# AlainSchoebi/semantic-bundle-adjustment-colmap

Hardware: AMD Instinct MI355X
Metric: residuals+Jacobians/sec and BA-iteration wall-time, 1k cams / 1M pts / 10M obs (higher is better)
Workload: dtype f64

## Files before the change

### semantic-bundle-adjustment-colmap_amd/csrc/semantic.hip

```cpp
#include <hip/hip_runtime.h>

#include <map>

#include <algorithm>
#include <cmath>
#include <cstring>
#include <type_traits>

#include "ba_math.h"
#include "kernels.h"
#include "semantic.h"
#include "step_bodies.h"

namespace miba {

namespace {

constexpr double kMinStep = 1.4901161193847656e-08;

struct SemArgs {
  const SemSample* samples;
  const SemPair* pairs;
  const double* qt;
  const double* cam;
// ... 147 lines not shown
  const double aa = a * a, bb = b * b, cc = c * c, dd = d * d;
  const double ab = a * b, ac = a * c, ad = a * d, bc = b * c, bd = b * d, cd = c * d;
  Q[0] = aa + bb - cc - dd; Q[1] = 2.0 * (bc - ad);  Q[2] = 2.0 * (ac + bd);
  Q[3] = 2.0 * (bc + ad);  Q[4] = aa - bb + cc - dd; Q[5] = 2.0 * (cd - ab);
  Q[6] = 2.0 * (bd - ac);  Q[7] = 2.0 * (ab + cd);  Q[8] = aa - bb - cc + dd;
}

[[maybe_unused]] __device__ inline double rcp_refined(double x) {
  double r = __builtin_amdgcn_rcp(x);
  r = fma(r, fma(-x, r, 1.0), r);
  r = fma(r, fma(-x, r, 1.0), r);
  return r;
}

template <int M>
__device__ inline double distortion_gain(const double* K, double r2) {
  constexpr int np = Model<M>::kNumParams;
  double s = 0.0;
  if constexpr (M == kSimpleRadial || M == kRadial) {
#pragma unroll
    for (int k = 3; k < np; ++k) s += fabs(K[k]);
  } else if constexpr (M == kOpenCV) {
#pragma unroll
    for (int k = 4; k < np; ++k) s += fabs(K[k]);
  }
  const double g = 1.0 + r2;
  return 1.0 + s * g * g * g;
}

template <int M>
__device__ inline void world_to_image_fma(const double* K, double u, double v, double* x, double* y) {
#pragma clang fp contract(fast)
  if constexpr (M == kSimplePinhole) {
    *x = K[0] * u + K[1];
    *y = K[0] * v + K[2];
  } else if constexpr (M == kPinhole) {
    *x = K[0] * u + K[2];
    *y = K[1] * v + K[3];
  } else if constexpr (M == kSimpleRadial || M == kRadial) {
    const double r2 = u * u + v * v;
    double rad = K[3] * r2;
    if constexpr (M == kRadial) rad = rad + K[4] * r2 * r2;
// ... 5 lines not shown
    const double rad = k1 * r2 + k2 * r2 * r2;
    const double du = u * rad + 2.0 * p1 * uv + p2 * (r2 + 2.0 * u2);
    const double dv = v * rad + 2.0 * p2 * uv + p1 * (r2 + 2.0 * v2);
    *x = K[0] * (u + du) + K[2];
    *y = K[1] * (v + dv) + K[3];
  }
}

__device__ inline void matvec3_t_fma(const double* A, double v0, double v1, double v2, const double* t,
                                     double pp[3]) {
#pragma clang fp contract(fast)
#pragma unroll
  for (int c = 0; c < 3; ++c) pp[c] = A[3 * c] * v0 + A[3 * c + 1] * v1 + A[3 * c + 2] * v2 + t[c];
}

template <int M>
__device__ inline double margin_model_term(const double* K2, const double p[3], double mag) {
  const double iz = 1.0 / p[2];
  const double u = p[0] * iz, v = p[1] * iz;
  return 2e-11 * (fabs(K2[0]) + fabs(K2[1])) * distortion_gain<M>(K2, u * u + v * v) * (1.0 + fabs(u) + fabs(v)) *
         (1.0 + mag * fabs(iz));
}

template <int M, bool FAST = false>
__device__ inline bool resolve(const SemArgs& a, const double p[3], double mag, float label1, const double* K2,
                               const float2* dl2, const PixelCache& pc, double& f, double exk = 0.0) {
  double iz;
  if constexpr (FAST) {
    const double x0 = p[2];
    double r = __builtin_amdgcn_rcp(x0);
    iz = fma(r, fma(-x0, r, 1.0), r);
  } else {
    iz = rcp_refined(p[2]);
  }
  const double u = p[0] * iz, v = p[1] * iz;
// ... 20 lines not shown
    f = 0.0;
    return true;
  }
  float2 s;
  if (pc.valid && px == pc.px && py == pc.py) {
    s = make_float2(pc.depth, pc.label);
  } else {
    s = dl2[(size_t)py * a.W + px];
  }
  const double dd = fabs((double)s.x - p[2]) - a.threshold;
  if (!(fabs(dd) > 1e-9 * (1.0 + fabs((double)s.x) + mag))) return false;
  f = (dd > 0.0) ? 0.0 : ((label1 == s.y) ? 0.0 : 1.0);
  return true;
}

struct PairConst {
  double q1[4], t1[3], q2[4], t2[3];
  double uqi[4];
  double ti[3];
  double u2[4];
  double R2[9];
  double C[9];
  double K2[8];
  uint32_t var1, var2, mask1, mask2;
  uint32_t slot, H2, W2, TW2;
  uint64_t roff, toff;
  double pert[28];
  double ood[14];
  double A[16][9];
  double pj[8][3];
  double rho1, rho2, dt1[3], dt2[3];
};

__device__ __forceinline__ SemArgs with_pair(const SemArgs& ak, const PairConst* __restrict__ P) {
  SemArgs a = ak;
  a.H = (int)P->H2;
  a.W = (int)P->W2;
  a.TW = (int)P->TW2;
  return a;
}

__device__ inline void stencil_bounds(const double* q, const double* t, double rel_step, double* rho, double dt[3]) {
  const double nq2 = q[0] * q[0] + q[1] * q[1] + q[2] * q[2] + q[3] * q[3];
  const double nq = sqrt(nq2);
  double r = 0.0;
  for (int k = 0; k < 4; ++k) {
    const double delta = fmax(kMinStep, fabs(q[k]) * rel_step);
    const double d = fmax(fabs((q[k] + delta) - q[k]), fabs(q[k] - (q[k] - delta)));
    const double perp = d * sqrt(fmax(0.0, 1.0 - q[k] * q[k] / nq2));
    const double den = nq - d;
    r = fmax(r, den > 0.0 ? 2.0 * perp / den : INFINITY);
  }
  *rho = r * 1.001;
  for (int k = 0; k < 3; ++k) {
    const double delta = fmax(kMinStep, fabs(t[k]) * rel_step);
    dt[k] = fmax(fabs((t[k] + delta) - t[k]), fabs(t[k] - (t[k] - delta))) * 1.001;
  }
}

__device__ inline void stencil_prep(const double* q1, const double* t1, const double* q2, const double* t2,
                                    double rel_step, int e, PairConst* __restrict__ P) {
  const int m = e >> 1;
  const bool minus = e & 1;
  const int grp = m < 4 ? 0 : (m < 7 ? 1 : (m < 11 ? 2 : 3));
  const int k = m - (grp == 0 ? 0 : (grp == 1 ? 4 : (grp == 2 ? 7 : 11)));
  const double orig = grp == 0 ? q1[k] : (grp == 1 ? t1[k] : (grp == 2 ? q2[k] : t2[k]));
  const double delta = fmax(kMinStep, fabs(orig) * rel_step);
  const double pert = minus ? orig - delta : orig + delta;
  P->pert[e] = pert;
  if (minus) {
    double one_over_delta = 1.0 / delta;
    one_over_delta /= 2;
// ... 28 lines not shown
      for (int kk = 1; kk < 4; ++kk) v = kk == k ? PJ[3 * kk + c] : v;
      P->pj[(grp == 0 ? 0 : 4) + k][c] = v;
    }
  }
}

constexpr int kPairVals = 78 + 12;
constexpr int kPairStride = 96;
constexpr int kSemRow = 13;

__device__ __forceinline__ void pair_prep_body(int k, int lane, const SemPair* __restrict__ pairs, int npairs,
                                      const double* __restrict__ qt, const double* __restrict__ cam,
                                      const uint32_t* __restrict__ img_cam, const uint32_t* __restrict__ img_flags,
                                      const uint32_t* __restrict__ raster_slot, const SlotInfo* __restrict__ slots,
                                      double rel_step, PairConst* __restrict__ out, double* __restrict__ pair_blk,
                                      int blk_stride, uint32_t* __restrict__ pair_cnt) {
  if (k >= npairs) return;
  for (int e = lane; e < blk_stride; e += 32) pair_blk[(size_t)k * blk_stride + e] = 0.0;
  if (pair_cnt && lane == 31) pair_cnt[k] = 0u;
  if (lane > 30) return;
  const SemPair pr = pairs[k];
  const double* a1 = qt + 8 * (size_t)pr.i;
  const double* a2 = qt + 8 * (size_t)pr.j;
  if (lane < 28) {
    stencil_prep(a1, a1 + 4, a2, a2 + 4, rel_step, lane, out + k);
    return;
  }
  PairConst& P = out[k];
  const double zero[3] = {0.0, 0.0, 0.0};
  if (lane == 28) {
    const double q1[4] = {a1[0], a1[1], a1[2], a1[3]}, t1[3] = {a1[4], a1[5], a1[6]};
    for (int m = 0; m < 4; ++m) P.q1[m] = q1[m];
    for (int m = 0; m < 3; ++m) P.t1[m] = t1[m];
    Pose1Stage s;
    pose1_stage(q1, zero, s);
    {
      const double sc = 1.0 / sqrt(q1[0] * q1[0] + q1[1] * q1[1] + q1[2] * q1[2] + q1[3] * q1[3]);
      const double qi[4] = {sc * q1[0], -(sc * q1[1]), -(sc * q1[2]), -(sc * q1[3])};
      const double scale = 1.0 / sqrt(qi[0] * qi[0] + qi[1] * qi[1] + qi[2] * qi[2] + qi[3] * qi[3]);
// ... 34 lines not shown
    double u2[4], R2[9];
    unit_quat(q2, u2);
    unit_quat_matrix(u2, R2);
    for (int r = 0; r < 3; ++r)
      for (int c = 0; c < 3; ++c)
        P.C[3 * r + c] = R2[3 * r] * s.R[c] + R2[3 * r + 1] * s.R[3 + c] + R2[3 * r + 2] * s.R[6 + c];
  }
}

__global__ void semantic_pair_prep_kernel(const SemPair* __restrict__ pairs, int npairs, const double* __restrict__ qt,
                                          const double* __restrict__ cam, const uint32_t* __restrict__ img_cam,
                                          const uint32_t* __restrict__ img_flags,
                                          const uint32_t* __restrict__ raster_slot,
                                          const SlotInfo* __restrict__ slots, double rel_step,
                                          PairConst* __restrict__ out, double* __restrict__ pair_blk, int blk_stride,
                                          uint32_t* __restrict__ pair_cnt, uint32_t* __restrict__ zero_n = nullptr,
                                          int nzero = 0) {
  if (zero_n && blockIdx.x == 0 && (int)threadIdx.x < nzero) zero_n[threadIdx.x] = 0u;
  pair_prep_body(blockIdx.x * 2 + (threadIdx.x >> 5), threadIdx.x & 31, pairs, npairs, qt, cam, img_cam, img_flags,
                 raster_slot, slots, rel_step, out, pair_blk, blk_stride, pair_cnt);
}

struct PrepArgs {
  const SemPair* pairs;
  int npairs;
  const double* qt;
  const double* cam;
  const uint32_t* img_cam;
  const uint32_t* img_flags;
  const uint32_t* raster_slot;
  const SlotInfo* slots;
  double rel_step;
  PairConst* out;
  double* pair_blk;
  uint32_t* pair_cnt;
  uint32_t* dcount;
};

template <int U>
__global__ __launch_bounds__(256, 8) void step_prologue_kernel(PrepArgs a, int nprep, DevProblem p,
                                                            double* __restrict__ rec, double* __restrict__ zero,
                                                            int nzero, int npack, TouchRanges t, unsigned* sink,
                                                            int nwarm) {
  const int b = blockIdx.x;
  if (b < nprep) {
    if (b == 0 && (int)threadIdx.x < kNumModels) a.dcount[threadIdx.x] = 0u;
    pair_prep_body(b * 8 + (threadIdx.x >> 5), threadIdx.x & 31, a.pairs, a.npairs, a.qt, a.cam, a.img_cam,
                   a.img_flags, a.raster_slot, a.slots, a.rel_step, a.out, a.pair_blk, kPairStride, a.pair_cnt);
  } else if (b < nprep + npack) {
    pack_image_record(p, rec, zero, nzero, (b - nprep) * 256 + (int)threadIdx.x);
  } else {
    touch_ranges<U>(t, sink, b - nprep - npack, nwarm);
  }
}


template <int M>
__device__ __forceinline__ double stencil_reference(const SemArgs& a, const PairConst* __restrict__ P, int grp, int k,
                                                 double pert, const double pc1[3], float label1, const double* K2,
                                                 const float2* dl2) {
  double qq1[4], tt1[3], qq2[4], tt2[3];
#pragma unroll
  for (int c = 0; c < 4; ++c) {
// ... 301 lines not shown
  }
  return ok;
}

struct Centre {
  double pw[3], p2[3], w[3];
  double r, mag, exk;
  PixelCache pc;
  int st;
};

template <int M, bool FAST>
__device__ __forceinline__ void centre_eval(const SemArgs& a, const PairConst* __restrict__ P, const SemSample& smp,
                                            const double* K2, const float2* dl2, Centre& c) {
  double rot[3];
  unit_quat_rotate(P->uqi, smp.pc1, rot);
  c.pw[0] = rot[0] + P->ti[0];
  c.pw[1] = rot[1] + P->ti[1];
  c.pw[2] = rot[2] + P->ti[2];
  double rot2[3];
  unit_quat_rotate(P->u2, c.pw, rot2);
  c.p2[0] = rot2[0] + P->t2[0];
  c.p2[1] = rot2[1] + P->t2[1];
  c.p2[2] = rot2[2] + P->t2[2];
  c.pc.valid = false;
  c.pc.px = c.pc.py = 0;
  c.pc.depth = c.pc.label = 0.f;
  c.st = 0;
  c.r = project_centre<M>(a, c.p2, smp.label1, K2, dl2, c.pc, &c.st);
  c.mag = fabs(smp.pc1[0]) + fabs(smp.pc1[1]) + fabs(smp.pc1[2]) + fabs(P->t1[0]) + fabs(P->t1[1]) +
          fabs(P->t1[2]) + fabs(c.pw[0]) + fabs(c.pw[1]) + fabs(c.pw[2]) + fabs(P->t2[0]) + fabs(P->t2[1]) +
          fabs(P->t2[2]);
  c.w[0] = smp.pc1[0] - P->t1[0];
  c.w[1] = smp.pc1[1] - P->t1[1];
  c.w[2] = smp.pc1[2] - P->t1[2];
  c.exk = FAST ? margin_model_term<M>(K2, c.p2, c.mag) : 0.0;
}

template <int M, bool FAST, int NB>
__device__ __forceinline__ bool stencil_full(const SemArgs& a, const PairConst* __restrict__ P, const Centre& c,
                                             const SemSample& smp, const double* K2, const float2* dl2,
                                             double Jt[12], const float2* box = nullptr,
                                             const FlatBox* fb = nullptr) {
  if constexpr (NB > 0) {
    const int cidx = c.pc.valid ? c.pc.py * a.W + c.pc.px : 0;
    if (!stencil_batched<M, FAST, NB>(a, P, c.w, c.pw, c.p2, c.mag, smp.label1, K2, dl2, cidx, c.exk, Jt, box, fb)) {
      stencil_rolled<M, FAST>(a, P, c.w, c.pw, c.p2, c.mag, smp.pc1, smp.label1, K2, dl2, c.pc, c.exk, Jt);
      return true;
    }
    return false;
  } else {
// ... 1 lines not shown
    return true;
  }
}


template <int M>
__device__ __forceinline__ double second_derivative_bound(const double* K, double rho) {
  if constexpr (M == kSimpleRadial) {
    return 6.0 * fabs(K[3]) * rho;
  } else if constexpr (M == kRadial) {
    return 6.0 * fabs(K[3]) * rho + 20.0 * fabs(K[4]) * rho * rho * rho;
  } else if constexpr (M == kOpenCV) {
    return 6.0 * fabs(K[4]) * rho + 20.0 * fabs(K[5]) * rho * rho * rho + 6.0 * (fabs(K[6]) + fabs(K[7]));
  } else {
    return 0.0;
  }
}

template <int M>
__device__ __forceinline__ bool flat_box(const PairConst* __restrict__ P, const Centre& c, const double* K2,
                                         FlatBox& fb) {
  const double z = c.p2[2];
  if (!(z > 0.0)) return false;
  const double iz = 1.0 / z;
  const double u = c.p2[0] * iz, v = c.p2[1] * iz;
  constexpr int np = Model<M>::kNumParams;
  double x, y, A[4], Jp[2 * np];
  world_to_image_jac<M>(K2, u, v, &x, &y, A, Jp);
  if (!(fabs(x) < 1e8 && fabs(y) < 1e8 && fabs(u) < 1e6 && fabs(v) < 1e6)) return false;
  const double dq1 = P->var1 ? P->rho1 * sqrt(c.w[0] * c.w[0] + c.w[1] * c.w[1] + c.w[2] * c.w[2]) * (1.0 + 1e-12) : 0.0;
// ... 38 lines not shown
  }
  const double gain = distortion_gain<M>(K2, u * u + v * v);
  const double kscale = (fabs(K2[0]) + fabs(K2[1])) * gain * (1.0 + fabs(u) + fabs(v)) * (1.0 + c.mag * fabs(iz));
  const double ex = 1e-6 + 1e-11 * (kscale + fabs(x) + fabs(y));
  const double bx = bxm * (1.0 + 1e-12) + ex;
  const double by = bym * (1.0 + 1e-12) + ex;
  fb.x0 = (int)round(x - bx);
  fb.y0 = (int)round(y - by);
  fb.ncol = (int)round(x + bx) - fb.x0 + 1;
  fb.nrow = (int)round(y + by) - fb.y0 + 1;
  fb.d = az_max;
  return fb.ncol <= 3 && fb.nrow <= 3;
}

template <int M>
__device__ __forceinline__ void image_jac_bound(const double* K, double u, double v, double Ah[4]) {
  const double r2 = u * u + v * v, r1 = fabs(u) + fabs(v);
  if constexpr (M == kSimplePinhole) {
    Ah[0] = Ah[3] = fabs(K[0]);
    Ah[1] = Ah[2] = 0.0;
  } else if constexpr (M == kPinhole) {
    Ah[0] = fabs(K[0]);
    Ah[3] = fabs(K[1]);
    Ah[1] = Ah[2] = 0.0;
  } else if constexpr (M == kSimpleRadial) {
    const double k = fabs(K[3]);
    Ah[0] = Ah[3] = fabs(K[0]) * (1.0 + 3.0 * k * r2);
    Ah[1] = Ah[2] = fabs(K[0]) * (k * r2);
  } else if constexpr (M == kRadial) {
    const double k1 = fabs(K[3]), k2 = fabs(K[4]);
    Ah[0] = Ah[3] = fabs(K[0]) * (1.0 + 3.0 * k1 * r2 + 5.0 * k2 * r2 * r2);
    Ah[1] = Ah[2] = fabs(K[0]) * (k1 * r2 + 2.0 * k2 * r2 * r2);
  } else {
    const double k1 = fabs(K[4]), k2 = fabs(K[5]), p1 = fabs(K[6]), p2 = fabs(K[7]);
    const double rad = 3.0 * k1 * r2 + 5.0 * k2 * r2 * r2, off = k1 * r2 + 2.0 * k2 * r2 * r2 + 2.0 * (p1 + p2) * r1;
    Ah[0] = fabs(K[0]) * (1.0 + rad + (2.0 * p1 + 6.0 * p2) * r1);
    Ah[1] = fabs(K[0]) * off;
    Ah[2] = fabs(K[1]) * off;
    Ah[3] = fabs(K[1]) * (1.0 + rad + (6.0 * p1 + 2.0 * p2) * r1);
  }
}

template <int M, bool EXACT_A = false, bool GROUPS = false>
__device__ __forceinline__ bool flat_box_coarse(const PairConst* __restrict__ P, const Centre& c, const double* K2,
                                                double u, double v, double x, double y, FlatBox& fb) {
  const double z = c.p2[2];
  if (!(z > 0.0)) return false;
  double Ae[4];
  if constexpr (EXACT_A) {
    constexpr int np = Model<M>::kNumParams;
    double Jp[2 * np];
    world_to_image_jac<M>(K2, u, v, &x, &y, Ae, Jp);
  }
  if (!(fabs(x) < 1e8 && fabs(y) < 1e8 && fabs(u) < 1e6 && fabs(v) < 1e6)) return false;
  double dq = 0.0, tx = 0.0, ty = 0.0, tz = 0.0;
  if (P->var1) {
    dq = P->rho1 * sqrt(c.w[0] * c.w[0] + c.w[1] * c.w[1] + c.w[2] * c.w[2]) * (1.0 + 1e-12);
    tx = fmax(P->dt1[0] * fabs(P->C[0]), fmax(P->dt1[1] * fabs(P->C[1]), P->dt1[2] * fabs(P->C[2])));
    ty = fmax(P->dt1[0] * fabs(P->C[3]), fmax(P->dt1[1] * fabs(P->C[4]), P->dt1[2] * fabs(P->C[5])));
    tz = fmax(P->dt1[0] * fabs(P->C[6]), fmax(P->dt1[1] * fabs(P->C[7]), P->dt1[2] * fabs(P->C[8])));
  }
  if (P->var2) {
    dq = fmax(dq, P->rho2 * sqrt(c.pw[0] * c.pw[0] + c.pw[1] * c.pw[1] + c.pw[2] * c.pw[2]) * (1.0 + 1e-12));
    tx = fmax(tx, P->dt2[0]);
    ty = fmax(ty, P->dt2[1]);
    tz = fmax(tz, P->dt2[2]);
  }
  const double az = fmax(dq, tz);
  if (!(z - az > 0.5 * z)) return false;
  const double iden = 1.0 / (z - az) * (1.0 + 1e-12);
  const double cu_r = (dq + fabs(u) * dq) * iden, cv_r = (dq + fabs(v) * dq) * iden;
  const double cu_t = (tx + fabs(u) * tz) * iden, cv_t = (ty + fabs(v) * tz) * iden;
  const double cu = fmax(cu_r, cu_t), cv = fmax(cv_r, cv_t);
  const double gm = fmax(cu, cv);
  if (!(gm < 0.1)) return false;
  const double ru = fabs(u) + gm, rv = fabs(v) + gm;
  const double H = second_derivative_bound<M>(K2, sqrt(ru * ru + rv * rv) * (1.0 + 1e-12));
  const double fx = fabs(K2[0]);
  const double fy = (M == kPinhole || M == kOpenCV) ? fabs(K2[1]) : fabs(K2[0]);
  double Ah[4];
  if constexpr (EXACT_A) {
#pragma unroll
    for (int k = 0; k < 4; ++k) Ah[k] = fabs(Ae[k]);
  } else {
    image_jac_bound<M>(K2, u, v, Ah);
  }
  double bxm, bym;
  if constexpr (GROUPS) {
    const double sr = cu_r + cv_r, st = cu_t + cv_t;
    bxm = fmax((Ah[0] + fx * H * sr) * cu_r + (Ah[1] + fx * H * sr) * cv_r,
               (Ah[0] + fx * H * st) * cu_t + (Ah[1] + fx * H * st) * cv_t);
    bym = fmax((Ah[2] + fy * H * sr) * cu_r + (Ah[3] + fy * H * sr) * cv_r,
               (Ah[2] + fy * H * st) * cu_t + (Ah[3] + fy * H * st) * cv_t);
  } else {
    const double sk = cu + cv;
    bxm = (Ah[0] + fx * H * sk) * cu + (Ah[1] + fx * H * sk) * cv;
    bym = (Ah[2] + fy * H * sk) * cu + (Ah[3] + fy * H * sk) * cv;
  }
  const double gain = distortion_gain<M>(K2, u * u + v * v);
  const double kscale = (fabs(K2[0]) + fabs(K2[1])) * gain * (1.0 + fabs(u) + fabs(v)) * (1.0 + c.mag * fabs(1.0 / z));
  const double ex = 1e-6 + 1e-11 * (kscale + fabs(x) + fabs(y));
  const double bx = bxm * (1.0 + 1e-12) + ex;
  const double by = bym * (1.0 + 1e-12) + ex;
  fb.x0 = (int)round(x - bx);
  fb.y0 = (int)round(y - by);
  fb.ncol = (int)round(x + bx) - fb.x0 + 1;
  fb.nrow = (int)round(y + by) - fb.y0 + 1;
  fb.d = az;
  return fb.ncol <= 3 && fb.nrow <= 3;
}

__device__ __forceinline__ int flat_index(const SemArgs& a, const FlatBox& fb, bool cand, int q) {
  const int px = fb.x0 + q % 3, py = fb.y0 + q / 3;
  const bool in = cand && q % 3 < fb.ncol && q / 3 < fb.nrow && px >= 0 && px < a.W && py >= 0 && py < a.H;
  return in ? py * a.W + px : 0;
// ... 270 lines not shown
  if (!(dmin <= dmax)) return 0;
  const double margin = fb.d + 1e-9 * (1.0 + fmax(fabs(dmin), fabs(dmax)) + mag);
  const double far = fmax(fabs(dmax - z), fabs(dmin - z));
  if (a.threshold - far > margin) return 1;
  const double nearest = (z >= dmin && z <= dmax) ? 0.0 : fmin(fabs(dmin - z), fabs(dmax - z));
  if (nearest - a.threshold > margin) return 2;
  return 0;
}

template <int M, bool WS, bool LP, int COARSE>
__device__ __forceinline__ double flat_sample(const SemArgs& a, const PairConst* __restrict__ P, const double* K2,
                                              const float2* dl2, const float* spal, const SemSample& smp, Centre& c,
                                              bool& deferred, bool& decided) {
  deferred = false;
  double rot[3];
  unit_quat_rotate(P->uqi, smp.pc1, rot);
  c.pw[0] = rot[0] + P->ti[0];
  c.pw[1] = rot[1] + P->ti[1];
  c.pw[2] = rot[2] + P->ti[2];
  double rot2[3];
  unit_quat_rotate(P->u2, c.pw, rot2);
  c.p2[0] = rot2[0] + P->t2[0];
  c.p2[1] = rot2[1] + P->t2[1];
  c.p2[2] = rot2[2] + P->t2[2];
  c.mag = fabs(smp.pc1[0]) + fabs(smp.pc1[1]) + fabs(smp.pc1[2]) + fabs(P->t1[0]) + fabs(P->t1[1]) +
          fabs(P->t1[2]) + fabs(c.pw[0]) + fabs(c.pw[1]) + fabs(c.pw[2]) + fabs(P->t2[0]) + fabs(P->t2[1]) +
          fabs(P->t2[2]);
  c.w[0] = smp.pc1[0] - P->t1[0];
  c.w[1] = smp.pc1[1] - P->t1[1];
  c.w[2] = smp.pc1[2] - P->t1[2];
  const double u2 = c.p2[0] / c.p2[2];
  const double v2 = c.p2[1] / c.p2[2];
  double x2, y2;
  world_to_image<M>(K2, u2, v2, &x2, &y2);
  const int cpx = cast_to_int_x86(round(x2));
  const int cpy = cast_to_int_x86(round(y2));
  const bool cin = !(cpx < 0 || cpx >= a.W || cpy < 0 || cpy >= a.H);
  FlatBox fb;
  const bool cand = COARSE == 3   ? flat_box_coarse<M, false, true>(P, c, K2, u2, v2, x2, y2, fb)
                    : COARSE == 2 ? flat_box_coarse<M, true>(P, c, K2, u2, v2, x2, y2, fb)
                    : COARSE == 1 ? flat_box_coarse<M>(P, c, K2, u2, v2, x2, y2, fb)
                                  : flat_box<M>(P, c, K2, fb);
  decided = false;
  bool resolved = false;
  if constexpr (LP) {
    if (cand && fb.x0 >= 0 && fb.y0 >= 0 && fb.x0 + fb.ncol <= a.W && fb.y0 + fb.nrow <= a.H && cpx >= fb.x0 &&
        cpx < fb.x0 + fb.ncol && cpy >= fb.y0 && cpy < fb.y0 + fb.nrow) {
      const float2 dr = a.dtile[P->toff + (size_t)(fb.y0 >> 3) * a.TW + (fb.x0 >> 3)];
      const uint8_t* lp = a.lab8 + P->roff + (size_t)fb.y0 * a.W + fb.x0;
// ... 35 lines not shown
    float2 s[9];
#pragma unroll
    for (int q = 0; q < 9; ++q) s[q] = dl2[flat_index(a, fb, cand, q)];
    if (!cin) {
      c.st = MI_BA_OUT_OF_BOUNDS;
      c.r = 0.0;
    } else if (fabs((double)sc.x - c.p2[2]) > a.threshold) {
      c.st = MI_BA_INVALID_DEPTH;
      c.r = 0.0;
    } else {
      c.st = MI_BA_VALID;
      c.r = (smp.label1 == sc.y) ? 0.0 : 1.0;
    }
    deferred = !(cand && flat_check(a, fb, s, c.p2[2], c.mag, smp.label1, c.r));
  }
  double rho[3];
  loss_eval(a.loss_type, a.loss_scale, c.r * c.r, rho);
  return 0.5 * (a.weight * rho[0]);
}

__device__ __forceinline__ void tile_cost_sum(double cost, double* sred, int tid, int lane, double* __restrict__ out) {
  double v = cost;
  for (int off = 32; off > 0; off >>= 1) v += __shfl_xor(v, off, 64);
  if (lane == 0) sred[tid >> 6] = v;
  __syncthreads();
  if (tid == 0) {
    double s = 0.0;
#pragma unroll
    for (int w = 0; w < kBlock / 64; ++w) s += sred[w];
    *out = s;
  }
}

// ... 124 lines not shown
        cb = 12;
      }
      double acc = 0.0;
      for (int q = 0; q < rows; ++q) acc += sJ[q * kSemRow + ca] * sJ[q * kSemRow + cb];
      cpart[((size_t)pair_chunk0[ch.x] + ch.y / 64) * kPairVals + e] = acc;
    }
  }
  __syncthreads();
  }
}

template <int M>
__device__ __forceinline__ void centre_geometry(const PairConst* __restrict__ P, const SemSample& smp,
                                                const double* K2, Centre& c) {
  double rot[3];
  unit_quat_rotate(P->uqi, smp.pc1, rot);
  c.pw[0] = rot[0] + P->ti[0];
  c.pw[1] = rot[1] + P->ti[1];
  c.pw[2] = rot[2] + P->ti[2];
  double rot2[3];
  unit_quat_rotate(P->u2, c.pw, rot2);
  c.p2[0] = rot2[0] + P->t2[0];
  c.p2[1] = rot2[1] + P->t2[1];
  c.p2[2] = rot2[2] + P->t2[2];
  c.pc.valid = false;
  c.pc.px = c.pc.py = 0;
  c.pc.depth = c.pc.label = 0.f;
  c.st = 0;
  c.r = 0.0;
  c.mag = fabs(smp.pc1[0]) + fabs(smp.pc1[1]) + fabs(smp.pc1[2]) + fabs(P->t1[0]) + fabs(P->t1[1]) +
          fabs(P->t1[2]) + fabs(c.pw[0]) + fabs(c.pw[1]) + fabs(c.pw[2]) + fabs(P->t2[0]) + fabs(P->t2[1]) +
          fabs(P->t2[2]);
  c.w[0] = smp.pc1[0] - P->t1[0];
  c.w[1] = smp.pc1[1] - P->t1[1];
  c.w[2] = smp.pc1[2] - P->t1[2];
  c.exk = margin_model_term<M>(K2, c.p2, c.mag);
}

template <int M, int GRP>
__device__ __forceinline__ bool stencil_group(const SemArgs& a, const PairConst* __restrict__ P, const Centre& c,
                                              const SemSample& smp, const double* K2, const float2* dl2,
                                              double col[3]) {
  constexpr int n = (GRP == 0 || GRP == 2) ? 4 : 3;
  constexpr int m0 = GRP == 0 ? 0 : (GRP == 1 ? 4 : (GRP == 2 ? 7 : 11));
  const uint32_t mask = GRP == 1 ? P->mask1 : (GRP == 3 ? P->mask2 : 0u);
  col[0] = col[1] = col[2] = 0.0;
  const PixelCache none = {0, 0, 0.f, 0.f, false};
  double fp[4], fm[4];
  const bool ok = stencil_step<M, true, GRP, 4>(a, P, m0, 0, n, c.w, c.pw, c.p2, c.mag, smp.label1, K2, dl2, 0, c.exk,
                                                fp, fm);
  if (ok) {
// ... 1079 lines not shown

void semantic_destroy(mi_ba_context* ctx) {
  if (!ctx->sem) return;
  delete ctx->sem;
  ctx->sem = nullptr;
}

mi_ba_status semantic_pair_prep(mi_ba_context* ctx, hipStream_t stream) {
  SemanticState* S = ctx->sem;
  if (!S || S->ns == 0 || S->npairs == 0) return MI_BA_OK;
  SemArgs a = make_args(ctx, ctx->dev.qt, ctx->dev.cam);
  PairConst* pcs = reinterpret_cast<PairConst*>(S->pconst.ptr);
  hipLaunchKernelGGL(semantic_pair_prep_kernel, dim3((S->npairs + 1) / 2), dim3(64), 0, stream, S->pairs.ptr,
                     S->npairs, a.qt, a.cam, a.img_cam, a.img_flags, a.raster_slot, a.slots, a.rel_step, pcs,
                     S->pair_blk.ptr,
                     kPairStride, ctx->sem_variant == 6 ? S->pair_cnt.ptr : nullptr,
                     ctx->sem_variant == 6 ? S->dcount.ptr : nullptr, kNumModels);
  return hipGetLastError() == hipSuccess ? MI_BA_OK : MI_BA_ERR_HIP;
}

mi_ba_status semantic_step_prologue(mi_ba_context* ctx, hipStream_t stream, double* zero, int nzero, unsigned* sink,
                                    int warm_mask, int warm_wgs, int warm_unroll) {
  SemanticState* S = ctx->sem;
  if (!S || S->ns == 0 || S->npairs == 0 || ctx->sem_variant != 6) return MI_BA_ERR_STATE;
  const DevProblem& d = ctx->dev;
  SemArgs a = make_args(ctx, d.qt, d.cam);
  PrepArgs pa{S->pairs.ptr, S->npairs, a.qt, a.cam, a.img_cam, a.img_flags, a.raster_slot, a.slots, a.rel_step,
              reinterpret_cast<PairConst*>(S->pconst.ptr), S->pair_blk.ptr, S->pair_cnt.ptr, S->dcount.ptr};
  const int nprep = (S->npairs + 7) / 8;
  const int npack = (int)((std::max<int64_t>(d.num_images, nzero) + 255) / 256);
  const int nwarm = touch_workgroups(warm_wgs);
  const TouchRanges t = touch_input_ranges(d, warm_mask);
  const dim3 grid((unsigned)(nprep + npack + nwarm));
  if (warm_unroll >= 8)
    hipLaunchKernelGGL(step_prologue_kernel<8>, grid, dim3(256), 0, stream, pa, nprep, d, ctx->img_rec.ptr, zero, nzero,
                       npack, t, sink, nwarm);
  else
    hipLaunchKernelGGL(step_prologue_kernel<4>, grid, dim3(256), 0, stream, pa, nprep, d, ctx->img_rec.ptr, zero, nzero,
                       npack, t, sink, nwarm);
  return hipGetLastError() == hipSuccess ? MI_BA_OK : MI_BA_ERR_HIP;
}

bool semantic_step_fusable(const mi_ba_context* ctx) {
// ... 294 lines not shown
```

Measured before the change: 20.32 billion.

## Precompute per-pair camera, rotation and loss constants in pair prep

Result: no change. 20.12 billion (-1.0%).

```diff
diff --git a/semantic-bundle-adjustment-colmap_amd/csrc/semantic.hip b/semantic-bundle-adjustment-colmap_amd/csrc/semantic.hip
--- a/semantic-bundle-adjustment-colmap_amd/csrc/semantic.hip
+++ b/semantic-bundle-adjustment-colmap_amd/csrc/semantic.hip
@@ -185,7 +185,7 @@
 }
 
 template <int M>
-__device__ inline double distortion_gain(const double* K, double r2) {
+__device__ inline double distortion_gain_sum(const double* K) {
   constexpr int np = Model<M>::kNumParams;
   double s = 0.0;
   if constexpr (M == kSimpleRadial || M == kRadial) {
@@ -195,8 +195,17 @@
 #pragma unroll
     for (int k = 4; k < np; ++k) s += fabs(K[k]);
   }
+  return s;
+}
+
+__device__ inline double distortion_gain_s(double s, double r2) {
   const double g = 1.0 + r2;
   return 1.0 + s * g * g * g;
+}
+
+template <int M>
+__device__ inline double distortion_gain(const double* K, double r2) {
+  return distortion_gain_s(distortion_gain_sum<M>(K), r2);
 }
 
 template <int M>
@@ -232,11 +241,10 @@
   for (int c = 0; c < 3; ++c) pp[c] = A[3 * c] * v0 + A[3 * c + 1] * v1 + A[3 * c + 2] * v2 + t[c];
 }
 
-template <int M>
-__device__ inline double margin_model_term(const double* K2, const double p[3], double mag) {
+__device__ inline double margin_model_term(const double* __restrict__ kf, const double p[3], double mag) {
   const double iz = 1.0 / p[2];
   const double u = p[0] * iz, v = p[1] * iz;
-  return 2e-11 * (fabs(K2[0]) + fabs(K2[1])) * distortion_gain<M>(K2, u * u + v * v) * (1.0 + fabs(u) + fabs(v)) *
+  return 2e-11 * kf[0] * distortion_gain_s(kf[1], u * u + v * v) * (1.0 + fabs(u) + fabs(v)) *
          (1.0 + mag * fabs(iz));
 }
 
@@ -287,22 +295,89 @@
   return true;
 }
 
+template <int M>
+__device__ inline void camera_terms(const double* K, double kf[5], double kd[5], double kj[6]) {
+  kf[0] = fabs(K[0]) + fabs(K[1]);
+  kf[1] = distortion_gain_sum<M>(K);
+  kf[2] = kf[3] = kf[4] = 0.0;
+#pragma unroll
+  for (int m = 0; m < 5; ++m) kd[m] = 0.0;
+#pragma unroll
+  for (int m = 0; m < 6; ++m) kj[m] = 0.0;
+  if constexpr (M == kSimpleRadial) {
+    kf[2] = 6.0 * fabs(K[3]);
+    kd[4] = 2.0 * K[3];
+    kj[0] = 3.0 * fabs(K[3]);
+  } else if constexpr (M == kRadial) {
+    kf[2] = 6.0 * fabs(K[3]);
+    kf[3] = 20.0 * fabs(K[4]);
+    kd[4] = 2.0 * K[4];
+    kj[0] = 3.0 * fabs(K[3]);
+    kj[1] = 5.0 * fabs(K[4]);
+    kj[2] = 2.0 * fabs(K[4]);
+  } else if constexpr (M == kOpenCV) {
+    const double p1 = fabs(K[6]), p2 = fabs(K[7]);
+    kf[2] = 6.0 * fabs(K[4]);
+    kf[3] = 20.0 * fabs(K[5]);
+    kf[4] = 6.0 * (p1 + p2);
+    kd[0] = 2.0 * K[6];
+    kd[1] = 2.0 * K[7];
+    kd[2] = 6.0 * K[6];
+    kd[3] = 6.0 * K[7];
+    kd[4] = 2.0 * K[5];
+    kj[0] = 3.0 * fabs(K[4]);
+    kj[1] = 5.0 * fabs(K[5]);
+    kj[2] = 2.0 * fabs(K[5]);
+    kj[3] = 2.0 * (p1 + p2);
+    kj[4] = 2.0 * p1 + 6.0 * p2;
+    kj[5] = 6.0 * p1 + 2.0 * p2;
+  }
+}
+
+__device__ inline void quat_rotate_sums(const double q[4], double s[9]) {
+  const double t2 = q[0] * q[1];
+  const double t3 = q[0] * q[2];
+  const double t4 = q[0] * q[3];
+  const double t5 = -(q[1] * q[1]);
+  const double t6 = q[1] * q[2];
+  const double t7 = q[1] * q[3];
+  const double t8 = -(q[2] * q[2]);
+  const double t9 = q[2] * q[3];
+  const double t1 = -(q[3] * q[3]);
+  s[0] = t8 + t1; s[1] = t6 - t4; s[2] = t3 + t7;
+  s[3] = t4 + t6; s[4] = t5 + t1; s[5] = t9 - t2;
+  s[6] = t7 - t3; s[7] = t2 + t9; s[8] = t5 + t8;
+}
+
+__device__ __forceinline__ void unit_quat_rotate_sums(const double* __restrict__ s, const double p[3], double r[3]) {
+  r[0] = 2.0 * (s[0] * p[0] + s[1] * p[1] + s[2] * p[2]) + p[0];
+  r[1] = 2.0 * (s[3] * p[0] + s[4] * p[1] + s[5] * p[2]) + p[1];
+  r[2] = 2.0 * (s[6] * p[0] + s[7] * p[1] + s[8] * p[2]) + p[2];
+}
+
 struct PairConst {
-  double q1[4], t1[3], q2[4], t2[3];
+  double t1[3], ti[3], t2[3];
+  double rs1[9], rs2[9];
+  double rho1, rho2;
+  double ft[3];
+  double kf[5];
+  double kd[5];
+  double K2[8];
+  double cost0, cost1;
+  uint32_t var1, var2, mask1, mask2;
+  uint32_t slot, H2, W2, TW2;
+  uint64_t roff, toff;
+  double kj[6];
+  double dt1[3], dt2[3];
+  double q1[4], q2[4];
   double uqi[4];
-  double ti[3];
   double u2[4];
   double R2[9];
   double C[9];
-  double K2[8];
-  uint32_t var1, var2, mask1, mask2;
-  uint32_t slot, H2, W2, TW2;
-  uint64_t roff, toff;
   double pert[28];
   double ood[14];
   double A[16][9];
   double pj[8][3];
-  double rho1, rho2, dt1[3], dt2[3];
 };
 
 __device__ __forceinline__ SemArgs with_pair(const SemArgs& ak, const PairConst* __restrict__ P) {
@@ -311,6 +386,13 @@
   a.W = (int)P->W2;
   a.TW = (int)P->TW2;
   return a;
+}
+
+__device__ inline void stencil_bounds_t(const double* t, double rel_step, double dt[3]) {
+  for (int k = 0; k < 3; ++k) {
+    const double delta = fmax(kMinStep, fabs(t[k]) * rel_step);
+    dt[k] = fmax(fabs((t[k] + delta) - t[k]), fabs(t[k] - (t[k] - delta))) * 1.001;
+  }
 }
 
 __device__ inline void stencil_bounds(const double* q, const double* t, double rel_step, double* rho, double dt[3]) {
@@ -325,10 +407,15 @@
     r = fmax(r, den > 0.0 ? 2.0 * perp / den : INFINITY);
   }
   *rho = r * 1.001;
-  for (int k = 0; k < 3; ++k) {
-    const double delta = fmax(kMinStep, fabs(t[k]) * rel_step);
-    dt[k] = fmax(fabs((t[k] + delta) - t[k]), fabs(t[k] - (t[k] - delta))) * 1.001;
-  }
+  stencil_bounds_t(t, rel_step, dt);
+}
+
+__device__ inline double flat_translation_bound(const double Cr[3], const double dt1[3], double dt2r, bool var1,
+                                                bool var2) {
+  double t = 0.0;
+  if (var1) t = fmax(dt1[0] * fabs(Cr[0]), fmax(dt1[1] * fabs(Cr[1]), dt1[2] * fabs(Cr[2])));
+  if (var2) t = fmax(t, dt2r);
+  return t;
 }
 
 __device__ inline void stencil_prep(const double* q1, const double* t1, const double* q2, const double* t2,
@@ -387,15 +474,65 @@
                                       const uint32_t* __restrict__ img_cam, const uint32_t* __restrict__ img_flags,
                                       const uint32_t* __restrict__ raster_slot, const SlotInfo* __restrict__ slots,
                                       double rel_step, PairConst* __restrict__ out, double* __restrict__ pair_blk,
-                                      int blk_stride, uint32_t* __restrict__ pair_cnt) {
+                                      int blk_stride, uint32_t* __restrict__ pair_cnt,
+                                      const uint8_t* __restrict__ cam_model, int loss_type, double loss_scale,
+                                      double weight) {
   if (k >= npairs) return;
   for (int e = lane; e < blk_stride; e += 32) pair_blk[(size_t)k * blk_stride + e] = 0.0;
   if (pair_cnt && lane == 31) pair_cnt[k] = 0u;
-  if (lane > 30) return;
   const SemPair pr = pairs[k];
+  if (lane == 31) {
+    PairConst& P = out[k];
+    const uint32_t c2 = img_cam[pr.j];
+    const double* K = cam + 8 * (size_t)c2;
+    switch_model(cam_model[c2], [&](auto m) { camera_terms<decltype(m)::value>(K, P.kf, P.kd, P.kj); });
+    double rho[3];
+    loss_eval(loss_type, loss_scale, 0.0 * 0.0, rho);
+    P.cost0 = 0.5 * (weight * rho[0]);
+    loss_eval(loss_type, loss_scale, 1.0 * 1.0, rho);
+    P.cost1 = 0.5 * (weight * rho[0]);
+    return;
+  }
   const double* a1 = qt + 8 * (size_t)pr.i;
   const double* a2 = qt + 8 * (size_t)pr.j;
   if (lane < 28) {
+    PairConst& P = out[k];
+    if (lane >= 8 && lane < 11) {
+      const int r = lane - 8;
+      const double zero[3] = {0.0, 0.0, 0.0};
+      double R2r[3], Cr[3];
+      {
+        double u2[4], R2[9];
+        unit_quat(a2, u2);
+        unit_quat_matrix(u2, R2);
+#pragma unroll
+        for (int c = 0; c < 3; ++c) R2r[c] = r == 0 ? R2[c] : (r == 1 ? R2[3 + c] : R2[6 + c]);
+      }
+      Pose1Stage s;
+      pose1_stage(a1, zero, s);
+#pragma unroll
+      for (int c = 0; c < 3; ++c) Cr[c] = R2r[0] * s.R[c] + R2r[1] * s.R[3 + c] + R2r[2] * s.R[6 + c];
+      double dt1[3], dt2[3];
+      stencil_bounds_t(a1 + 4, rel_step, dt1);
+      stencil_bounds_t(a2 + 4, rel_step, dt2);
+      const double dt2r = r == 0 ? dt2[0] : (r == 1 ? dt2[1] : dt2[2]);
+      P.ft[r] = flat_translation_bound(Cr, dt1, dt2r, pr.var1 != 0, pr.var2 != 0);
+    } else if (lane == 22) {
+      const double sc = 1.0 / sqrt(a1[0] * a1[0] + a1[1] * a1[1] + a1[2] * a1[2] + a1[3] * a1[3]);
+      const double qi[4] = {sc * a1[0], -(sc * a1[1]), -(sc * a1[2]), -(sc * a1[3])};
+      const double scale = 1.0 / sqrt(qi[0] * qi[0] + qi[1] * qi[1] + qi[2] * qi[2] + qi[3] * qi[3]);
+      const double uqi[4] = {scale * qi[0], scale * qi[1], scale * qi[2], scale * qi[3]};
+      double rs[9];
+      quat_rotate_sums(uqi, rs);
+#pragma unroll
+      for (int m = 0; m < 9; ++m) P.rs1[m] = rs[m];
+    } else if (lane == 23) {
+      double u2[4], rs[9];
+      unit_quat(a2, u2);
+      quat_rotate_sums(u2, rs);
+#pragma unroll
+      for (int m = 0; m < 9; ++m) P.rs2[m] = rs[m];
+    }
     stencil_prep(a1, a1 + 4, a2, a2 + 4, rel_step, lane, out + k);
     return;
   }
@@ -460,11 +597,13 @@
                                           const uint32_t* __restrict__ raster_slot,
                                           const SlotInfo* __restrict__ slots, double rel_step,
                                           PairConst* __restrict__ out, double* __restrict__ pair_blk, int blk_stride,
-                                          uint32_t* __restrict__ pair_cnt, uint32_t* __restrict__ zero_n = nullptr,
-                                          int nzero = 0) {
+                                          uint32_t* __restrict__ pair_cnt, const uint8_t* __restrict__ cam_model,
+                                          int loss_type, double loss_scale, double weight,
+                                          uint32_t* __restrict__ zero_n = nullptr, int nzero = 0) {
   if (zero_n && blockIdx.x == 0 && (int)threadIdx.x < nzero) zero_n[threadIdx.x] = 0u;
   pair_prep_body(blockIdx.x * 2 + (threadIdx.x >> 5), threadIdx.x & 31, pairs, npairs, qt, cam, img_cam, img_flags,
-                 raster_slot, slots, rel_step, out, pair_blk, blk_stride, pair_cnt);
+                 raster_slot, slots, rel_step, out, pair_blk, blk_stride, pair_cnt, cam_model, loss_type, loss_scale,
+                 weight);
 }
 
 struct PrepArgs {
@@ -481,6 +620,9 @@
   double* pair_blk;
   uint32_t* pair_cnt;
   uint32_t* dcount;
+  const uint8_t* cam_model;
+  int loss_type;
+  double loss_scale, weight;
 };
 
 template <int U>
@@ -492,7 +634,8 @@
   if (b < nprep) {
     if (b == 0 && (int)threadIdx.x < kNumModels) a.dcount[threadIdx.x] = 0u;
     pair_prep_body(b * 8 + (threadIdx.x >> 5), threadIdx.x & 31, a.pairs, a.npairs, a.qt, a.cam, a.img_cam,
-                   a.img_flags, a.raster_slot, a.slots, a.rel_step, a.out, a.pair_blk, kPairStride, a.pair_cnt);
+                   a.img_flags, a.raster_slot, a.slots, a.rel_step, a.out, a.pair_blk, kPairStride, a.pair_cnt,
+                   a.cam_model, a.loss_type, a.loss_scale, a.weight);
   } else if (b < nprep + npack) {
     pack_image_record(p, rec, zero, nzero, (b - nprep) * 256 + (int)threadIdx.x);
   } else {
@@ -824,12 +967,12 @@
 __device__ __forceinline__ void centre_eval(const SemArgs& a, const PairConst* __restrict__ P, const SemSample& smp,
                                             const double* K2, const float2* dl2, Centre& c) {
   double rot[3];
-  unit_quat_rotate(P->uqi, smp.pc1, rot);
+  unit_quat_rotate_sums(P->rs1, smp.pc1, rot);
   c.pw[0] = rot[0] + P->ti[0];
   c.pw[1] = rot[1] + P->ti[1];
   c.pw[2] = rot[2] + P->ti[2];
   double rot2[3];
-  unit_quat_rotate(P->u2, c.pw, rot2);
+  unit_quat_rotate_sums(P->rs2, c.pw, rot2);
   c.p2[0] = rot2[0] + P->t2[0];
   c.p2[1] = rot2[1] + P->t2[1];
   c.p2[2] = rot2[2] + P->t2[2];
@@ -844,7 +987,7 @@
   c.w[0] = smp.pc1[0] - P->t1[0];
   c.w[1] = smp.pc1[1] - P->t1[1];
   c.w[2] = smp.pc1[2] - P->t1[2];
-  c.exk = FAST ? margin_model_term<M>(K2, c.p2, c.mag) : 0.0;
+  c.exk = FAST ? margin_model_term(P->kf, c.p2, c.mag) : 0.0;
 }
 
 template <int M, bool FAST, int NB>
@@ -876,6 +1019,74 @@
     return 6.0 * fabs(K[4]) * rho + 20.0 * fabs(K[5]) * rho * rho * rho + 6.0 * (fabs(K[6]) + fabs(K[7]));
   } else {
     return 0.0;
+  }
+}
+
+template <int M>
+__device__ __forceinline__ double second_derivative_bound_kf(const double* __restrict__ kf, double rho) {
+  if constexpr (M == kSimpleRadial) {
+    return kf[2] * rho;
+  } else if constexpr (M == kRadial) {
+    return kf[2] * rho + kf[3] * rho * rho * rho;
+  } else if constexpr (M == kOpenCV) {
+    return kf[2] * rho + kf[3] * rho * rho * rho + kf[4];
+  } else {
+    return 0.0;
+  }
+}
+
+template <int M>
+__device__ __forceinline__ void world_to_image_kd(const double* K, const double* __restrict__ kd, double u, double v,
+                                                  double* x, double* y) {
+  if constexpr (M == kOpenCV) {
+    const double k1 = K[4], k2 = K[5], p1 = K[6], p2 = K[7];
+    const double u2 = u * u, uv = u * v, v2 = v * v, r2 = u2 + v2;
+    const double radial = k1 * r2 + k2 * r2 * r2;
+    const double du = u * radial + kd[0] * uv + p2 * (r2 + 2.0 * u2);
+    const double dv = v * radial + kd[1] * uv + p1 * (r2 + 2.0 * v2);
+    const double xd = u + du, yd = v + dv;
+    *x = K[0] * xd + K[2];
+    *y = K[1] * yd + K[3];
+  } else {
+    world_to_image<M>(K, u, v, x, y);
+  }
+}
+
+template <int M>
+__device__ __forceinline__ void image_jac_kd(const double* K, const double* __restrict__ kd, double u, double v,
+                                             double A[4]) {
+  if constexpr (M == kSimplePinhole) {
+    A[0] = K[0]; A[1] = 0.0; A[2] = 0.0; A[3] = K[0];
+  } else if constexpr (M == kPinhole) {
+    A[0] = K[0]; A[1] = 0.0; A[2] = 0.0; A[3] = K[1];
+  } else if constexpr (M == kSimpleRadial) {
+    const double f = K[0], k = K[3];
+    const double u2 = u * u, v2 = v * v, r2 = u2 + v2;
+    const double radial = k * r2;
+    const double two_k_uv = kd[4] * u * v;
+    A[0] = f * (1.0 + radial + kd[4] * u2);
+    A[1] = f * two_k_uv;
+    A[2] = f * two_k_uv;
+    A[3] = f * (1.0 + radial + kd[4] * v2);
+  } else if constexpr (M == kRadial) {
+    const double f = K[0], k1 = K[3], k2 = K[4];
+    const double u2 = u * u, v2 = v * v, r2 = u2 + v2;
+    const double radial = k1 * r2 + k2 * r2 * r2;
+    const double g = 2.0 * (k1 + kd[4] * r2);
+    A[0] = f * (1.0 + radial + g * u2);
+    A[1] = f * (g * u * v);
+    A[2] = f * (g * u * v);
+    A[3] = f * (1.0 + radial + g * v2);
+  } else {
+    static_assert(M == kOpenCV, "the semantic term's five camera models");
+    const double fx = K[0], fy = K[1], k1 = K[4], k2 = K[5];
+    const double u2 = u * u, uv = u * v, v2 = v * v, r2 = u2 + v2;
+    const double radial = k1 * r2 + k2 * r2 * r2;
+    const double g = 2.0 * (k1 + kd[4] * r2);
+    A[0] = fx * (1.0 + radial + g * u2 + kd[0] * v + kd[3] * u);
+    A[1] = fx * (g * uv + kd[0] * u + kd[1] * v);
+    A[2] = fy * (g * uv + kd[1] * v + kd[0] * u);
+    A[3] = fy * (1.0 + radial + g * v2 + kd[1] * u + kd[2] * v);
   }
 }
 
@@ -944,7 +1155,8 @@
 }
 
 template <int M>
-__device__ __forceinline__ void image_jac_bound(const double* K, double u, double v, double Ah[4]) {
+__device__ __forceinline__ void image_jac_bound(const double* K, const double* __restrict__ kj, double u, double v,
+                                                double Ah[4]) {
   const double r2 = u * u + v * v, r1 = fabs(u) + fabs(v);
   if constexpr (M == kSimplePinhole) {
     Ah[0] = Ah[3] = fabs(K[0]);
@@ -955,19 +1167,19 @@
     Ah[1] = Ah[2] = 0.0;
   } else if constexpr (M == kSimpleRadial) {
     const double k = fabs(K[3]);
-    Ah[0] = Ah[3] = fabs(K[0]) * (1.0 + 3.0 * k * r2);
+    Ah[0] = Ah[3] = fabs(K[0]) * (1.0 + kj[0] * r2);
     Ah[1] = Ah[2] = fabs(K[0]) * (k * r2);
   } else if constexpr (M == kRadial) {
-    const double k1 = fabs(K[3]), k2 = fabs(K[4]);
-    Ah[0] = Ah[3] = fabs(K[0]) * (1.0 + 3.0 * k1 * r2 + 5.0 * k2 * r2 * r2);
-    Ah[1] = Ah[2] = fabs(K[0]) * (k1 * r2 + 2.0 * k2 * r2 * r2);
+    const double k1 = fabs(K[3]);
+    Ah[0] = Ah[3] = fabs(K[0]) * (1.0 + kj[0] * r2 + kj[1] * r2 * r2);
+    Ah[1] = Ah[2] = fabs(K[0]) * (k1 * r2 + kj[2] * r2 * r2);
   } else {
-    const double k1 = fabs(K[4]), k2 = fabs(K[5]), p1 = fabs(K[6]), p2 = fabs(K[7]);
-    const double rad = 3.0 * k1 * r2 + 5.0 * k2 * r2 * r2, off = k1 * r2 + 2.0 * k2 * r2 * r2 + 2.0 * (p1 + p2) * r1;
-    Ah[0] = fabs(K[0]) * (1.0 + rad + (2.0 * p1 + 6.0 * p2) * r1);
+    const double k1 = fabs(K[4]);
+    const double rad = kj[0] * r2 + kj[1] * r2 * r2, off = k1 * r2 + kj[2] * r2 * r2 + kj[3] * r1;
+    Ah[0] = fabs(K[0]) * (1.0 + rad + kj[4] * r1);
     Ah[1] = fabs(K[0]) * off;
     Ah[2] = fabs(K[1]) * off;
-    Ah[3] = fabs(K[1]) * (1.0 + rad + (6.0 * p1 + 2.0 * p2) * r1);
+    Ah[3] = fabs(K[1]) * (1.0 + rad + kj[5] * r1);
   }
 }
 
@@ -977,25 +1189,13 @@
   const double z = c.p2[2];
   if (!(z > 0.0)) return false;
   double Ae[4];
-  if constexpr (EXACT_A) {
-    constexpr int np = Model<M>::kNumParams;
-    double Jp[2 * np];
-    world_to_image_jac<M>(K2, u, v, &x, &y, Ae, Jp);
-  }
+  if constexpr (EXACT_A) image_jac_kd<M>(K2, P->kd, u, v, Ae);
   if (!(fabs(x) < 1e8 && fabs(y) < 1e8 && fabs(u) < 1e6 && fabs(v) < 1e6)) return false;
-  double dq = 0.0, tx = 0.0, ty = 0.0, tz = 0.0;
-  if (P->var1) {
-    dq = P->rho1 * sqrt(c.w[0] * c.w[0] + c.w[1] * c.w[1] + c.w[2] * c.w[2]) * (1.0 + 1e-12);
-    tx = fmax(P->dt1[0] * fabs(P->C[0]), fmax(P->dt1[1] * fabs(P->C[1]), P->dt1[2] * fabs(P->C[2])));
-    ty = fmax(P->dt1[0] * fabs(P->C[3]), fmax(P->dt1[1] * fabs(P->C[4]), P->dt1[2] * fabs(P->C[5])));
-    tz = fmax(P->dt1[0] * fabs(P->C[6]), fmax(P->dt1[1] * fabs(P->C[7]), P->dt1[2] * fabs(P->C[8])));
-  }
-  if (P->var2) {
+  double dq = 0.0;
+  if (P->var1) dq = P->rho1 * sqrt(c.w[0] * c.w[0] + c.w[1] * c.w[1] + c.w[2] * c.w[2]) * (1.0 + 1e-12);
+  if (P->var2)
     dq = fmax(dq, P->rho2 * sqrt(c.pw[0] * c.pw[0] + c.pw[1] * c.pw[1] + c.pw[2] * c.pw[2]) * (1.0 + 1e-12));
-    tx = fmax(tx, P->dt2[0]);
-    ty = fmax(ty, P->dt2[1]);
-    tz = fmax(tz, P->dt2[2]);
-  }
+  const double tx = P->ft[0], ty = P->ft[1], tz = P->ft[2];
   const double az = fmax(dq, tz);
   if (!(z - az > 0.5 * z)) return false;
   const double iden = 1.0 / (z - az) * (1.0 + 1e-12);
@@ -1005,7 +1205,7 @@
   const double gm = fmax(cu, cv);
   if (!(gm < 0.1)) return false;
   const double ru = fabs(u) + gm, rv = fabs(v) + gm;
-  const double H = second_derivative_bound<M>(K2, sqrt(ru * ru + rv * rv) * (1.0 + 1e-12));
+  const double H = second_derivative_bound_kf<M>(P->kf, sqrt(ru * ru + rv * rv) * (1.0 + 1e-12));
   const double fx = fabs(K2[0]);
   const double fy = (M == kPinhole || M == kOpenCV) ? fabs(K2[1]) : fabs(K2[0]);
   double Ah[4];
@@ -1013,7 +1213,7 @@
 #pragma unroll
     for (int k = 0; k < 4; ++k) Ah[k] = fabs(Ae[k]);
   } else {
-    image_jac_bound<M>(K2, u, v, Ah);
+    image_jac_bound<M>(K2, P->kj, u, v, Ah);
   }
   double bxm, bym;
   if constexpr (GROUPS) {
@@ -1027,8 +1227,8 @@
     bxm = (Ah[0] + fx * H * sk) * cu + (Ah[1] + fx * H * sk) * cv;
     bym = (Ah[2] + fy * H * sk) * cu + (Ah[3] + fy * H * sk) * cv;
   }
-  const double gain = distortion_gain<M>(K2, u * u + v * v);
-  const double kscale = (fabs(K2[0]) + fabs(K2[1])) * gain * (1.0 + fabs(u) + fabs(v)) * (1.0 + c.mag * fabs(1.0 / z));
+  const double gain = distortion_gain_s(P->kf[1], u * u + v * v);
+  const double kscale = P->kf[0] * gain * (1.0 + fabs(u) + fabs(v)) * (1.0 + c.mag * fabs(1.0 / z));
   const double ex = 1e-6 + 1e-11 * (kscale + fabs(x) + fabs(y));
   const double bx = bxm * (1.0 + 1e-12) + ex;
   const double by = bym * (1.0 + 1e-12) + ex;
@@ -1329,12 +1529,12 @@
                                               bool& deferred, bool& decided) {
   deferred = false;
   double rot[3];
-  unit_quat_rotate(P->uqi, smp.pc1, rot);
+  unit_quat_rotate_sums(P->rs1, smp.pc1, rot);
   c.pw[0] = rot[0] + P->ti[0];
   c.pw[1] = rot[1] + P->ti[1];
   c.pw[2] = rot[2] + P->ti[2];
   double rot2[3];
-  unit_quat_rotate(P->u2, c.pw, rot2);
+  unit_quat_rotate_sums(P->rs2, c.pw, rot2);
   c.p2[0] = rot2[0] + P->t2[0];
   c.p2[1] = rot2[1] + P->t2[1];
   c.p2[2] = rot2[2] + P->t2[2];
@@ -1347,7 +1547,7 @@
   const double u2 = c.p2[0] / c.p2[2];
   const double v2 = c.p2[1] / c.p2[2];
   double x2, y2;
-  world_to_image<M>(K2, u2, v2, &x2, &y2);
+  world_to_image_kd<M>(K2, P->kd, u2, v2, &x2, &y2);
   const int cpx = cast_to_int_x86(round(x2));
   const int cpy = cast_to_int_x86(round(y2));
   const bool cin = !(cpx < 0 || cpx >= a.W || cpy < 0 || cpy >= a.H);
@@ -1413,9 +1613,7 @@
     }
     deferred = !(cand && flat_check(a, fb, s, c.p2[2], c.mag, smp.label1, c.r));
   }
-  double rho[3];
-  loss_eval(a.loss_type, a.loss_scale, c.r * c.r, rho);
-  return 0.5 * (a.weight * rho[0]);
+  return c.r == 0.0 ? P->cost0 : P->cost1;
 }
 
 __device__ __forceinline__ void tile_cost_sum(double cost, double* sred, int tid, int lane, double* __restrict__ out) {
@@ -1570,12 +1768,12 @@
 __device__ __forceinline__ void centre_geometry(const PairConst* __restrict__ P, const SemSample& smp,
                                                 const double* K2, Centre& c) {
   double rot[3];
-  unit_quat_rotate(P->uqi, smp.pc1, rot);
+  unit_quat_rotate_sums(P->rs1, smp.pc1, rot);
   c.pw[0] = rot[0] + P->ti[0];
   c.pw[1] = rot[1] + P->ti[1];
   c.pw[2] = rot[2] + P->ti[2];
   double rot2[3];
-  unit_quat_rotate(P->u2, c.pw, rot2);
+  unit_quat_rotate_sums(P->rs2, c.pw, rot2);
   c.p2[0] = rot2[0] + P->t2[0];
   c.p2[1] = rot2[1] + P->t2[1];
   c.p2[2] = rot2[2] + P->t2[2];
@@ -1590,7 +1788,7 @@
   c.w[0] = smp.pc1[0] - P->t1[0];
   c.w[1] = smp.pc1[1] - P->t1[1];
   c.w[2] = smp.pc1[2] - P->t1[2];
-  c.exk = margin_model_term<M>(K2, c.p2, c.mag);
+  c.exk = margin_model_term(P->kf, c.p2, c.mag);
 }
 
 template <int M, int GRP>
@@ -2700,8 +2898,8 @@
   hipLaunchKernelGGL(semantic_pair_prep_kernel, dim3((S->npairs + 1) / 2), dim3(64), 0, stream, S->pairs.ptr,
                      S->npairs, a.qt, a.cam, a.img_cam, a.img_flags, a.raster_slot, a.slots, a.rel_step, pcs,
                      S->pair_blk.ptr,
-                     kPairStride, ctx->sem_variant == 6 ? S->pair_cnt.ptr : nullptr,
-                     ctx->sem_variant == 6 ? S->dcount.ptr : nullptr, kNumModels);
+                     kPairStride, ctx->sem_variant == 6 ? S->pair_cnt.ptr : nullptr, a.cam_model, a.loss_type,
+                     a.loss_scale, a.weight, ctx->sem_variant == 6 ? S->dcount.ptr : nullptr, kNumModels);
   return hipGetLastError() == hipSuccess ? MI_BA_OK : MI_BA_ERR_HIP;
 }
 
@@ -2712,7 +2910,8 @@
   const DevProblem& d = ctx->dev;
   SemArgs a = make_args(ctx, d.qt, d.cam);
   PrepArgs pa{S->pairs.ptr, S->npairs, a.qt, a.cam, a.img_cam, a.img_flags, a.raster_slot, a.slots, a.rel_step,
-              reinterpret_cast<PairConst*>(S->pconst.ptr), S->pair_blk.ptr, S->pair_cnt.ptr, S->dcount.ptr};
+              reinterpret_cast<PairConst*>(S->pconst.ptr), S->pair_blk.ptr, S->pair_cnt.ptr, S->dcount.ptr,
+              a.cam_model, a.loss_type, a.loss_scale, a.weight};
   const int nprep = (S->npairs + 7) / 8;
   const int npack = (int)((std::max<int64_t>(d.num_images, nzero) + 255) / 256);
   const int nwarm = touch_workgroups(warm_wgs);
```
